# 10XGenomics/supernova

Measured on AMD Instinct MI355X. Metric: Gk-mers/s through count+graph at k=48, 1.2B×150bp; bit-exact counts, higher is better.
Workload: dtype u64

## Files before the change

### supernova_amd/csrc/snk_local.hip

```cpp
#include <string.h>
#include <cstring>
#include <rocprim/rocprim.hpp>

#include <type_traits>

#include "snk_ctx.h"
#include "snk_common.h"
#include "snk_kernels.h"
#include "snk_graph.h"
#include "snk_stages.h"

namespace {

constexpr uint32_t NONE = 0xFFFFFFFFu;
constexpr unsigned long long NONE64 = ~0ull;
constexpr uint16_t NONE16 = 0xFFFFu;
constexpr int TB = 256;

struct chunk_src {
    const uint32_t* chunk_n;
    const uint32_t* chunk_base;
    const uint4* extra;
    const unsigned long long* region_off;
    uint32_t NB, n_extra, n_regions;
    const uint8_t* span;
};
struct chunk_t {
    uint32_t bucket, n, lg, id;
    uint32_t span;
    uint64_t base;
};
struct bl_regions {
    const snk_u128* keys_r;
    const uint64_t* vals_r;
    const uint64_t* desc_src;
    snk_u128* keys_dense;
};
struct bl_shard {
    uint32_t bucket_base, NBl, me;
    uint32_t G;
    uint8_t* premote;
};
__global__ void __launch_bounds__(256) bl_chunk_merge_kernel(const uint32_t* __restrict__ chunk_n, const uint32_t* __restrict__ chunk_base, uint32_t NB, uint32_t G,
                                                             uint32_t cap, uint8_t* __restrict__ span, uint32_t* __restrict__ merged) {
    const uint32_t r = blockIdx.x * 256 + threadIdx.x;
    if (r >= G) return;
    uint32_t head = NONE, total = 0, m = 0, expect = 0;
    for (uint32_t b = r; b < NB; b += G) {
        const uint32_t n = chunk_n[b];
        span[b] = 1;
        merged[b] = n;
        if (n == 0) { head = NONE; continue; }
        const uint32_t base = chunk_base[b];
        if (head != NONE && base == expect && total + n <= cap && m < 255u) {
            total += n; ++m;
            merged[head] = total; merged[b] = 0; span[head] = (uint8_t)m;
        } else { head = b; total = n; m = 1; }
        expect = base + n;
    }
}
__global__ void __launch_bounds__(256) bl_chunk_desc_kernel(chunk_src cs, uint32_t nchunks, uint4* __restrict__ desc, uint64_t region_cap, uint64_t* __restrict__ desc_src) {
    const uint32_t c = blockIdx.x * 256 + threadIdx.x;
    if (c >= nchunks) return;
    uint32_t bucket, n, off = 0, meta = 0, region;
    if (c < cs.NB) {
        bucket = c; n = cs.chunk_n[c];
        if (n) off = cs.chunk_base[c];
        region = bucket % cs.n_regions;
        if (cs.span && n && cs.span[c] > 1) meta = 0x80000000u | cs.span[c];
    } else {
        const uint4 e = cs.extra[c - cs.NB];
        bucket = e.x; off = e.y; n = e.z & 0xFFFu; region = e.z >> 12; meta = e.w;
    }
    const uint64_t base = cs.region_off[region] + off;
    desc[c] = make_uint4((uint32_t)base, n, bucket, meta);
    if (desc_src) desc_src[c] = (uint64_t)region * region_cap + off;
}
__device__ __forceinline__ chunk_t chunk_get(const uint4* __restrict__ desc, uint32_t c) {
    const uint4 d = desc[c];
    chunk_t k;
    k.base = d.x; k.n = d.y; k.bucket = d.z; k.lg = d.w >> 24; k.id = d.w & 0xFFFFFFu; k.span = 1;
    if (d.w >> 31) { k.lg = 0; k.id = 0; k.span = d.w & 0xFFFFu; }
    return k;
}

__device__ __forceinline__ snk_kmer load_key(const snk_u128* keys, uint64_t i) {
    const uint64_t* p = reinterpret_cast<const uint64_t*>(keys + i);
    snk_kmer k;
    k.lo = p[0];
    k.hi = p[1];
    return k;
}
__device__ __forceinline__ uint32_t lhash(uint64_t hi, uint64_t lo) {
    uint32_t x = (uint32_t)(hi >> 32) * 0x9E3779B1u ^ (uint32_t)hi * 0x85EBCA77u ^ (uint32_t)(lo >> 32) * 0xC2B2AE3Du ^
                 (uint32_t)lo * 0x27D4EB2Fu;
    return snk_mix32(x);
}
template <int K>
__device__ __forceinline__ uint32_t oriented_base(snk_kmer k, bool rc, int idx) {
    return rc ? (snk_kmer_base<K>(k, K - 1 - idx) ^ 3u) : snk_kmer_base<K>(k, idx);
}

constexpr int BL_SPEC_LDS = 128;
constexpr int BL_SPEC_REPL = 64;
constexpr uint32_t BL_SPEC_BINS = 65536u;
constexpr uint32_t BL_SPEC_OVER = BL_SPEC_BINS + BL_SPEC_REPL * BL_SPEC_LDS / 2;
constexpr uint32_t BL_SPEC_WORDS = BL_SPEC_OVER + 16;
__global__ void __launch_bounds__(BL_SPEC_LDS) bl_spec_fold_kernel(unsigned long long* __restrict__ spec) {
    const uint32_t* rep = reinterpret_cast<const uint32_t*>(spec + BL_SPEC_BINS);
    unsigned long long s = 0;
    for (int r = 0; r < BL_SPEC_REPL; ++r) s += rep[r * BL_SPEC_LDS + threadIdx.x];
    spec[threadIdx.x] += s;
}
template <int K, int CAP, int T, bool BIG, bool GR, int MM>
__device__ __forceinline__ void bl_prune_chunk(const uint32_t c, const uint4* __restrict__ desc, uint32_t NB, bl_shard sh, const bl_regions& rg,
                                                     const snk_u128* __restrict__ keys, const uint64_t* __restrict__ vals,
                                                     uint32_t do_prune, uint8_t* __restrict__ ctx_out,
                                                     uint32_t* __restrict__ count_out, uint8_t* __restrict__ pend_out,
                                                     uint32_t* __restrict__ nbr_out, uint32_t* __restrict__ nbnd,
                                                     uint32_t* __restrict__ biglist, uint32_t* __restrict__ nbig,
                                                     unsigned long long* __restrict__ gindex, uint64_t gmask,
                                                     unsigned long long* __restrict__ spec, uint32_t* __restrict__ shist) {
    constexpr int HT = CAP <= 256 ? 512 : 4096;
    typedef typename std::conditional<(K <= 48 && !GR), uint32_t, uint64_t>::type klo_w;
    constexpr int KLS = (K <= 48 && !GR) ? 32 : 0;
    __shared__ uint64_t khi[CAP];
    __shared__ klo_w klo[CAP];
    __shared__ uint32_t ht[HT];
    __shared__ uint32_t bcnt;
    const int tid = threadIdx.x;
    const chunk_t ch = chunk_get(desc, c);
    if (ch.n == 0) return;
    if (!BIG && ch.n > (uint32_t)CAP) {
        if (tid == 0) biglist[atomicAdd(nbig, 1u)] = c;
        return;
    }
    const uint32_t n = ch.n;
    uint64_t src = ch.base;
    if (rg.keys_r) { src = rg.desc_src[c]; keys = rg.keys_r; vals = rg.vals_r; }
    __syncthreads();
    for (int s = tid; s < HT; s += T) ht[s] = 0;
    if (tid == 0) bcnt = 0;
    constexpr int NPT = (CAP + T - 1) / T;
    uint64_t myv[NPT];
    snk_kmer kq[NPT];
#pragma unroll
    for (int q = 0; q < NPT; ++q) {
        const uint32_t i = tid + q * T;
        myv[q] = 0;
        if (i < n) {
            kq[q] = load_key(keys, src + i);
            myv[q] = vals[src + i];
        }
    }
#pragma unroll
    for (int q = 0; q < NPT; ++q) {
        const uint32_t i = tid + q * T;
        if (i < n) {
            khi[i] = kq[q].hi;
            klo[i] = (klo_w)(kq[q].lo >> KLS);
            if (rg.keys_r) { uint64_t* d = reinterpret_cast<uint64_t*>(rg.keys_dense + ch.base + i); d[0] = kq[q].lo; d[1] = kq[q].hi; }
        }
    }
    __syncthreads();
    for (uint32_t i = tid; i < n; i += T) {
        uint32_t slot = lhash(khi[i], (uint64_t)klo[i] << KLS) & (HT - 1);
        for (;;) {
            const uint32_t old = atomicCAS(&ht[slot], 0u, i + 1u);
            if (old == 0u) break;
            slot = (slot + 1) & (HT - 1);
        }
    }
    __syncthreads();
    const uint32_t split_mask = (1u << ch.lg) - 1u;
    uint32_t mybnd = 0;
    __shared__ uint16_t mlist[8 * T];
    __shared__ uint32_t resL[T];
    __shared__ uint32_t mcnt;
#pragma unroll
    for (int q = 0; q < NPT; ++q) {
        const uint32_t i0 = q * T;
        if (i0 >= n) break;
        const uint32_t i = i0 + tid;
        const bool act = i < n;
        snk_kmer k;
        k.hi = act ? khi[i] : 0ull;
        k.lo = act ? ((uint64_t)klo[i] << KLS) : 0ull;
        uint64_t tag = 0;
        if (GR) { tag = k.lo & 0xFFFFFFFFull; k.lo &= ~0xFFFFFFFFull; }
        const uint64_t v = myv[q];
        const uint32_t c0 = (uint32_t)(v & 0xFFu);
        uint32_t keep = 0, miss = 0, nb0 = NONE, nb1 = NONE;
        const snk_kmer kr = snk_kmer_rc<K>(k);
        for (uint32_t rem = c0; rem; rem &= rem - 1) {
            const uint32_t bit = __ffs(rem) - 1;
            const snk_kmer y = bit < 4 ? snk_kmer_succ<K>(k, bit) : snk_kmer_pred<K>(k, bit - 4);
            const snk_kmer r = bit < 4 ? snk_kmer_pred<K>(kr, 3u - bit) : snk_kmer_succ<K>(kr, 7u - bit);
            const bool rev = snk_kmer_lt(r, y);
            snk_kmer cy = rev ? r : y;
            if (GR) cy.lo |= tag;
            int32_t j = -1;
            uint32_t slot = lhash(cy.hi, cy.lo) & (HT - 1);
            for (;;) {
                const uint32_t e = ht[slot];
                if (e == 0u) break;
                if (khi[e - 1] == cy.hi && ((uint64_t)klo[e - 1] << KLS) == cy.lo) { j = (int32_t)(e - 1); break; }
                slot = (slot + 1) & (HT - 1);
            }
            if (j >= 0) {
                keep |= 1u << bit;
                if (bit < 4) nb0 = ((uint32_t)j << 1) | (rev ? 1u : 0u); else nb1 = ((uint32_t)j << 1) | (rev ? 1u : 0u);
            } else miss |= 1u << bit;
        }
        if (tid == 0) mcnt = 0;
        resL[tid] = 0;
        __syncthreads();
        uint32_t pos = snk_wave_alloc(&mcnt, (uint32_t)__popc(miss));
        if (miss) {
            for (uint32_t bit = 0; bit < 8; ++bit)
                if (miss & (1u << bit)) mlist[pos++] = (uint16_t)((tid << 3) | bit);
        }
        __syncthreads();
        const uint32_t nm = mcnt;
        constexpr int SH = K - MM;
        constexpr int PER = (SH + 3) / 4;
        for (uint32_t it0 = 0; it0 < nm; it0 += T / 4) {
            const uint32_t item = it0 + (tid >> 2), sub = tid & 3u;
            const bool on = item < nm;
            const uint32_t ent = on ? mlist[item] : 0u;
            const uint32_t th = ent >> 3, bit = ent & 7u;
            const uint32_t ni = i0 + th;
            snk_kmer kk;
            kk.hi = on ? khi[ni] : 0ull;
            kk.lo = on ? ((uint64_t)klo[ni] << KLS) : 0ull;
            uint64_t ktag = 0;
            if (GR) { ktag = kk.lo & 0xFFFFFFFFull; kk.lo &= ~0xFFFFFFFFull; }
            const int first = bit < 4 ? 1 : 0;
            uint32_t mk = 0xFFFFFFFFu;
            for (int t = 0; t < PER; ++t) {
                const int sp = (int)sub * PER + t;
                if (sp < SH) {
                    const int pp = first + sp;
                    uint64_t w;
                    if (pp == 0) w = kk.hi;
                    else if (pp < 32) w = (kk.hi << (2 * pp)) | (kk.lo >> (64 - 2 * pp));
                    else if (pp == 32) w = kk.lo;
                    else w = kk.lo << (2 * pp - 64);
                    const uint32_t key = snk_mmer_key_top<MM>(w);
                    mk = key < mk ? key : mk;
                }
            }
            { const uint32_t o = __shfl_xor(mk, 1); mk = o < mk ? o : mk; }
            { const uint32_t o = __shfl_xor(mk, 2); mk = o < mk ? o : mk; }
            if (on && sub == 0) {
                const snk_kmer y = bit < 4 ? snk_kmer_succ<K>(kk, bit) : snk_kmer_pred<K>(kk, bit - 4);
                uint64_t wn;
                if (bit < 4) {
                    constexpr int pl = K - MM;
                    wn = pl < 32 ? ((y.hi << (2 * pl)) | (y.lo >> (64 - 2 * pl))) : (pl == 32 ? y.lo : (y.lo << (2 * pl - 64)));
                } else wn = y.hi;
                const uint32_t nkey = snk_mmer_key_top<MM>(wn);
                if (nkey < mk) mk = nkey;
                const uint32_t gb = snk_bucket_of_key(mk ^ (GR ? snk_group_mix((uint32_t)ktag) : 0u), NB);
                const uint32_t db = gb - (sh.bucket_base + ch.bucket);
                bool here = ch.span == 1 ? db == 0u : (gb >= sh.bucket_base + ch.bucket && db % sh.G == 0u && db / sh.G < ch.span);
                const bool remote = sh.NBl && gb / sh.NBl != sh.me;
                if (here && ch.lg) {
                    const snk_kmer r = snk_kmer_rc<K>(y);
                    snk_kmer cn = snk_kmer_lt(r, y) ? r : y;
                    if (GR) cn.lo |= ktag;
                    uint32_t h1, h2;
                    snk_kmer_hash_count<(K > 48) || GR>(cn, &h1, &h2);
                    here = (h2 & split_mask) == ch.id;
                }
                if (here && !(do_prune & 2u)) { if (!(do_prune & 1u)) atomicOr(&resL[th], 1u << bit); }
                else atomicOr(&resL[th], (1u << bit) | (0x100u << bit) | (remote ? (0x10000u << bit) : 0u));
            }
        }
        __syncthreads();
        const uint32_t res = resL[tid];
        keep |= res & 0xFFu;
        const uint32_t pm = (res >> 8) & 0xFFu;
        __syncthreads();
        if (!act) continue;
        const uint64_t gi = ch.base + i;
        ctx_out[gi] = (uint8_t)keep;
        pend_out[gi] = (uint8_t)pm;
        if (sh.premote) sh.premote[gi] = (uint8_t)(res >> 16);
        const uint32_t cnt = (uint32_t)(v >> 8);
        count_out[gi] = cnt;
        if (spec) {
            const uint32_t sc = cnt > 0xFFFFFFu ? 0xFFFFFFu : cnt;
            if (sc < (uint32_t)BL_SPEC_LDS) atomicAdd(&shist[sc], 1u);
            else if (sc < BL_SPEC_BINS) atomicAdd(&spec[sc], 1ull);
            else spec[BL_SPEC_OVER] = 1ull;
        }
        nbr_out[gi] = (nb0 == NONE ? 0x0FFFu : nb0) | (snk_kmer_eq(k, kr) ? 0x8000u : 0u) | ((nb1 == NONE ? 0x0FFFu : nb1) << 16);
        if (pm) {
            ++mybnd;
            if (gindex) {
                snk_kmer kk;
                kk.hi = khi[i];
                kk.lo = (uint64_t)klo[i] << KLS;
                uint32_t h1, h2;
                snk_kmer_hash2(kk, &h1, &h2);
                uint64_t slot = (((uint64_t)h1 << 32) | h2) & gmask;
                const unsigned long long ent = ((unsigned long long)h1 << 32) | (unsigned long long)(gi + 1);
                if (gindex[gmask + 1] == 0ull) {
                    bool placed = false;
                    for (uint32_t tries = 0; tries < 64; ++tries) {
                        const unsigned long long old = atomicCAS(&gindex[slot], 0ull, ent);
                        if (old == 0ull) { placed = true; break; }
                        slot = (slot + 1) & gmask;
                    }
                    if (!placed) gindex[gmask + 1] = 1ull;
                }
            }
        }
    }
    snk_wave_add(&bcnt, mybnd);
    __syncthreads();
    if (tid == 0) nbnd[c] = bcnt;
}
template <int K, int CAP, int T, bool BIG, bool GR, int MM>
__global__ void __launch_bounds__(T) bl_prune_kernel(const uint4* __restrict__ desc, uint32_t NB, bl_shard sh, bl_regions rg, const uint32_t* __restrict__ biglist_in,
                                                     uint32_t nchunks, uint32_t cpw,
                                                     const snk_u128* __restrict__ keys, const uint64_t* __restrict__ vals,
                                                     uint32_t do_prune, uint8_t* __restrict__ ctx_out,
                                                     uint32_t* __restrict__ count_out, uint8_t* __restrict__ pend_out,
                                                     uint32_t* __restrict__ nbr_out, uint32_t* __restrict__ nbnd,
                                                     uint32_t* __restrict__ biglist, uint32_t* __restrict__ nbig, const uint32_t* __restrict__ n_dev,
                                                     unsigned long long* __restrict__ gindex, uint64_t gmask, unsigned long long* __restrict__ spec) {
    __shared__ uint32_t shist[BL_SPEC_LDS];
    if (spec) {
        for (int j = threadIdx.x; j < BL_SPEC_LDS; j += T) shist[j] = 0;
        __syncthreads();
    }
    if (BIG && n_dev) {
        const uint32_t nb = *n_dev;
        for (uint32_t w = blockIdx.x; w < nb; w += gridDim.x)
            bl_prune_chunk<K, CAP, T, BIG, GR, MM>(biglist_in[w], desc, NB, sh, rg, keys, vals, do_prune, ctx_out, count_out, pend_out, nbr_out, nbnd, biglist, nbig, gindex, gmask,
                                                   spec, shist);
    } else {
        for (uint32_t r = 0; r < cpw; ++r) {
            const uint32_t w = blockIdx.x * cpw + r;
            if (w >= nchunks) break;
            bl_prune_chunk<K, CAP, T, BIG, GR, MM>(BIG ? biglist_in[w] : w, desc, NB, sh, rg, keys, vals, do_prune, ctx_out, count_out, pend_out, nbr_out,
                                           nbnd, biglist, nbig, gindex, gmask, spec, shist);
        }
    }
    if (spec) {
        __syncthreads();
        uint32_t* rep = reinterpret_cast<uint32_t*>(spec + BL_SPEC_BINS) + (blockIdx.x % BL_SPEC_REPL) * BL_SPEC_LDS;
        for (int j = threadIdx.x; j < BL_SPEC_LDS; j += T)
            if (shist[j]) atomicAdd(&rep[j], shist[j]);
    }
}

__global__ void __launch_bounds__(TB) bl_index_build_kernel(const snk_u128* __restrict__ keys, const uint8_t* __restrict__ pend,
                                                            uint64_t n, unsigned long long* __restrict__ tab, uint64_t mask) {
    const uint64_t i = (uint64_t)blockIdx.x * TB + threadIdx.x;
    if (i >= n || !pend[i]) return;
    const snk_kmer k = load_key(keys, i);
    uint32_t h1, h2;
    snk_kmer_hash2(k, &h1, &h2);
    uint64_t slot = (((uint64_t)h1 << 32) | h2) & mask;
    const unsigned long long ent = ((unsigned long long)h1 << 32) | (unsigned long long)(i + 1);
    for (;;) {
        const unsigned long long old = atomicCAS(&tab[slot], 0ull, ent);
        if (old == 0ull) break;
        slot = (slot + 1) & mask;
    }
}
template <int K, bool GR>
__global__ void __launch_bounds__(TB) bl_resolve_kernel(const snk_u128* __restrict__ keys, const uint8_t* __restrict__ pend,
                                                        uint64_t n, const unsigned long long* __restrict__ tab, uint64_t mask,
                                                        uint32_t do_prune, uint8_t* __restrict__ ctx, uint32_t* __restrict__ rq,
                                                        const uint8_t* __restrict__ premote) {
    constexpr int SPAN = 8 * TB;
    __shared__ uint16_t list[SPAN];
    __shared__ uint32_t cnt;
    const uint64_t base = (uint64_t)blockIdx.x * SPAN;
    if (threadIdx.x == 0) cnt = 0;
    __syncthreads();
    {
        const uint64_t i8 = base + 8ull * threadIdx.x;
        unsigned long long w = 0;
        if (i8 + 8 <= n) w = *reinterpret_cast<const unsigned long long*>(pend + i8);
        else for (uint64_t q = i8; q < n; ++q) w |= (unsigned long long)pend[q] << (8 * (q - i8));
        if (w) {
            uint32_t m = 0;
            for (int q = 0; q < 8; ++q) if ((w >> (8 * q)) & 0xFFull) ++m;
            uint32_t pos = atomicAdd(&cnt, m);
            for (int q = 0; q < 8; ++q) if ((w >> (8 * q)) & 0xFFull) list[pos++] = (uint16_t)(8 * threadIdx.x + q);
        }
    }
    __syncthreads();
    const uint32_t m = cnt;
    for (uint32_t it = threadIdx.x; it < m; it += TB) {
        const uint64_t i = base + list[it];
        const uint32_t pm = pend[i] & (premote ? ~(uint32_t)premote[i] : 0xFFu);
        snk_kmer k = load_key(keys, i);
        uint64_t tag = 0;
        if (GR) { tag = k.lo & 0xFFFFFFFFull; k.lo &= ~0xFFFFFFFFull; }
        uint32_t c = ctx[i];
        const snk_kmer kr = snk_kmer_rc<K>(k);
        for (uint32_t rem = pm; rem; rem &= rem - 1) {
            const uint32_t bit = __ffs(rem) - 1;
            const snk_kmer y = bit < 4 ? snk_kmer_succ<K>(k, bit) : snk_kmer_pred<K>(k, bit - 4);
            const snk_kmer r = bit < 4 ? snk_kmer_pred<K>(kr, 3u - bit) : snk_kmer_succ<K>(kr, 7u - bit);
            const bool rev = snk_kmer_lt(r, y);
            snk_kmer cy = rev ? r : y;
            if (GR) cy.lo |= tag;
            uint32_t h1, h2;
            snk_kmer_hash2(cy, &h1, &h2);
            uint64_t slot = (((uint64_t)h1 << 32) | h2) & mask;
            int64_t j = -1;
            for (;;) {
                const unsigned long long e = tab[slot];
                if (e == 0ull) break;
                if ((uint32_t)(e >> 32) == h1) {
                    const uint64_t idx = (uint32_t)e - 1u;
                    if (snk_kmer_eq(load_key(keys, idx), cy)) { j = (int64_t)idx; break; }
                }
                slot = (slot + 1) & mask;
            }
            if (j >= 0) rq[2 * i + (bit >> 2)] = ((uint32_t)j << 1) | (rev ? 1u : 0u);
            else if (do_prune) c &= ~(1u << bit);
            else rq[2 * i + (bit >> 2)] = NONE;
        }
        ctx[i] = (uint8_t)c;
    }
}

struct bl_extra_pool {
    unsigned long long* cur;
    uint64_t f0, b0;
    uint64_t fcap, bcap;
};
struct bl_dist_args {
    const uint8_t* premote;
    const uint32_t* rq_idx;
    const uint16_t* rq_meta;
    const unsigned long long* node_off;
    unsigned long long my_node_off;
};
template <int K, int CAP, int T, bool BIG, bool EMIT, bool DIST, bool GR>
__global__ void __launch_bounds__(T) bl_frag_kernel(const uint4* __restrict__ desc, const uint32_t* __restrict__ biglist_in,
                                                    const snk_u128* __restrict__ keys, const uint8_t* __restrict__ ctx,
                                                    const uint8_t* __restrict__ pend, const uint32_t* __restrict__ nbr,
                                                    const uint32_t* __restrict__ rq, bl_dist_args da, uint32_t* __restrict__ nfrag,
                                                    const uint32_t* __restrict__ foff, const uint64_t* __restrict__ boff,
                                                    uint32_t* __restrict__ nk, unsigned long long* __restrict__ hl_self,
                                                    unsigned long long* __restrict__ hl_nb, uint64_t* __restrict__ bstart,
                                                    uint8_t* __restrict__ fbases, uint32_t* __restrict__ fgroup, uint32_t* __restrict__ sfrag, bl_extra_pool xp) {
    constexpr int SPT = (2 * CAP + T - 1) / T;
    constexpr int NPT = (CAP + T - 1) / T;
    constexpr bool ONEW = T == 64;
    typedef typename std::conditional<(K <= 48 && !GR), uint32_t, uint64_t>::type klo_w;
    constexpr int KLS = (K <= 48 && !GR) ? 32 : 0;
    __shared__ uint64_t khi[ONEW ? 1 : CAP];
    __shared__ klo_w klo[ONEW ? 1 : CAP];
    __shared__ uint16_t nbL[2 * CAP];
    typedef typename std::conditional<(CAP <= 256), uint32_t, uint64_t>::type wrec_t;
    constexpr int FB = CAP <= 256 ? 10 : 16;
    constexpr uint32_t FM = (1u << FB) - 1u;
    __shared__ uint16_t lnk[2 * CAP];
    __shared__ wrec_t wr[2 * CAP];
    constexpr bool WIDE = (uint32_t)CAP * (uint32_t)K > 65535u;
    uint16_t* foffL = nbL;
    __shared__ uint32_t frel[WIDE ? CAP : 1];
    __shared__ uint16_t hnode[CAP];
    __shared__ uint8_t ctxL[CAP], pendL[CAP];
    __shared__ uint32_t fcnt, bcnt, changed;
    const int tid = threadIdx.x;
    const uint32_t c = BIG ? biglist_in[blockIdx.x] : blockIdx.x;
    const chunk_t ch = chunk_get(desc, c);
    if (ch.n == 0) return;
    if (!BIG && ch.n > (uint32_t)CAP) return;
    const uint32_t n = ch.n;
    const uint32_t c_foff = EMIT ? foff[c] : 0u;
    const uint64_t c_boff = EMIT ? boff[c] : 0ull;
    if constexpr (!ONEW) {
        if (tid == 0) { fcnt = 0; bcnt = 0; changed = 0; }
    }
    uint32_t w_frags = 0, w_bases = 0;
    snk_kmer kq[NPT] = {};
    {
        uint32_t cq[NPT], pq[NPT];
        uint32_t nq[NPT];
#pragma unroll
        for (int q = 0; q < NPT; ++q) {
            const uint32_t i = tid + q * T;
            if (i < n) {
                const uint64_t gi = ch.base + i;
                if (EMIT) kq[q] = load_key(keys, gi);
                cq[q] = ctx[gi];
                pq[q] = pend[gi];
                nq[q] = nbr[gi];
            }
        }
#pragma unroll
        for (int q = 0; q < NPT; ++q) {
            const uint32_t i = tid + q * T;
            if (i < n) {
                if constexpr (EMIT && !ONEW) {
                    const snk_kmer k = kq[q];
                    khi[i] = k.hi;
                    klo[i] = (klo_w)(k.lo >> KLS);
                }
                ctxL[i] = (uint8_t)cq[q];
                pendL[i] = (uint8_t)pq[q];
                nbL[2 * i] = (uint16_t)(nq[q] & 0x8FFFu);
                nbL[2 * i + 1] = (uint16_t)((nq[q] >> 16) & 0x0FFFu);
            }
        }
    }
    __syncthreads();
    auto is_pal = [&](uint32_t i) -> bool { return (nbL[2 * i] >> 15) != 0; };
    auto key_of = [&](uint32_t i) -> snk_kmer {
        snk_kmer k;
        if constexpr (ONEW) {
            k = load_key(keys, ch.base + i);
            k.lo = (k.lo >> KLS) << KLS;
        } else {
            k.hi = khi[i];
            k.lo = (uint64_t)klo[i] << KLS;
        }
        return k;
    };
    auto own_key = [&](int q, uint32_t i) -> snk_kmer {
        if constexpr (ONEW) return kq[q];
        else return key_of(i);
    };
    uint32_t myterm = 0;
    for (uint32_t s = tid; s < 2 * n; s += T) {
        const uint32_t i = s >> 1, side = s & 1u;
        const uint32_t cc = ctxL[i];
        const uint32_t bits = side ? (cc >> 4) : (cc & 15u);
        uint16_t out = NONE16;
        if (__popc(bits) == 1) {
            const uint32_t b = __ffs(bits) - 1;
            if (!((pendL[i] >> (4 * side + b)) & 1u)) {
                const uint32_t nb = nbL[s] & 0x0FFFu;
                if (nb != 0x0FFFu) {
                    const uint32_t j = nb >> 1, rev = nb & 1u;
                    const uint32_t fs = side ^ 1u ^ rev;
                    const uint32_t cj = ctxL[j];
                    const uint32_t deg = fs ? __popc(cj & 0xF0u) : __popc(cj & 0x0Fu);
                    if (deg == 1 && !is_pal(i) && !is_pal(j)) out = (uint16_t)((j << 1) | fs);
                }
            }
        }
        lnk[s] = out;
        if (!EMIT) { if (out == NONE16) ++myterm; }
        else if (out == NONE16) wr[s] = (wrec_t)FM | ((wrec_t)s << (2 * FB));
        else wr[s] = (wrec_t)(out ^ 1u) | ((wrec_t)1 << FB) | ((wrec_t)(out ^ 1u) << (2 * FB));
    }
    if (!EMIT) {
        if constexpr (ONEW) {
            const uint32_t total = (uint32_t)__builtin_amdgcn_readlane((int)snk_wave_scan_incl(myterm), 63);
            if (tid == 0) nfrag[c] = total >> 1;
        } else {
            snk_wave_add(&fcnt, myterm);
            __syncthreads();
            if (tid == 0) nfrag[c] = fcnt >> 1;
        }
        return;
    }
    __syncthreads();
    int max_rounds = 2;
    while ((1u << (max_rounds - 1)) < 2 * n) ++max_rounds;
    for (int round = 0; round < max_rounds; ++round) {
        wrec_t rr[SPT];
        bool any = false;
#pragma unroll
        for (int q = 0; q < SPT; ++q) {
            if ((uint32_t)(q * T) >= 2 * n) break;
            const uint32_t s = tid + q * T;
            if (s < 2 * n) {
                const wrec_t a0 = wr[s];
                const uint32_t n1 = (uint32_t)a0 & FM;
                rr[q] = a0;
                if (n1 != FM) {
                    const wrec_t a1 = wr[n1];
                    const uint32_t d = (((uint32_t)(a0 >> FB) & FM) + ((uint32_t)(a1 >> FB) & FM)) & FM;
                    rr[q] = (a1 & (wrec_t)FM) | ((wrec_t)d << FB) | (a1 & ((wrec_t)FM << (2 * FB)));
                    any = true;
                }
            }
        }
        if constexpr (ONEW) {
            if (!__any(any)) break;
        }
        __syncthreads();
#pragma unroll
        for (int q = 0; q < SPT; ++q) {
            if ((uint32_t)(q * T) >= 2 * n) break;
            const uint32_t s = tid + q * T;
            if (s < 2 * n) wr[s] = rr[q];
        }
        if constexpr (ONEW) {
            __syncthreads();
        } else {
            if (any) changed = 1;
            __syncthreads();
            const bool go = changed != 0;
            __syncthreads();
            if (tid == 0) changed = 0;
            if (!go) break;
        }
    }
    __syncthreads();
    auto w_next = [&](uint32_t st) -> uint32_t { return (uint32_t)wr[st] & FM; };
    auto w_dist = [&](uint32_t st) -> uint32_t { return (uint32_t)(wr[st] >> FB) & FM; };
    auto w_tail = [&](uint32_t st) -> uint32_t { return (uint32_t)(wr[st] >> (2 * FB)) & FM; };

    auto half_link = [&](uint32_t s) -> unsigned long long {
        const uint32_t i = s >> 1, side = s & 1u;
        const uint32_t cc = ctxL[i];
        const uint32_t bits = side ? (cc >> 4) : (cc & 15u);
        if (__popc(bits) != 1 || is_pal(i)) return NONE64;
        const uint32_t b = __ffs(bits) - 1;
        if (!((pendL[i] >> (4 * side + b)) & 1u)) return NONE64;
        snk_kmer k = key_of(i);
        if (GR) k.lo &= ~0xFFFFFFFFull;
        const snk_kmer y = side ? snk_kmer_pred<K>(k, b) : snk_kmer_succ<K>(k, b);
        if (snk_kmer_eq(y, snk_kmer_rc<K>(y))) return NONE64;
// ... 627 lines not shown
```

Baseline: 101.2.

## Shrink prune kernel LDS and registers for single-wave blocks to raise occupancy

For non-BIG 64-thread blocks, the local hash table now stores 16-bit indices (half the LDS), and the miss list is capped at 128 entries and processed in batches. Wave-level scans replace shared-memory atomic counters. Values are now streamed one iteration ahead instead of held in a per-thread array, and a waves_per_eu attribute asks the compiler to keep register use low enough for higher occupancy. The costs are a read-then-CAS loop on packed 16-bit slots, extra batch loops when misses exceed the list cap, and possible register spills from the occupancy constraint.

Result: faster. 102.5 (median of 6 runs) (+1.3%).

```diff
diff --git a/supernova_amd/csrc/snk_local.hip b/supernova_amd/csrc/snk_local.hip
--- a/supernova_amd/csrc/snk_local.hip
+++ b/supernova_amd/csrc/snk_local.hip
@@ -124,9 +124,11 @@
     constexpr int HT = CAP <= 256 ? 512 : 4096;
     typedef typename std::conditional<(K <= 48 && !GR), uint32_t, uint64_t>::type klo_w;
     constexpr int KLS = (K <= 48 && !GR) ? 32 : 0;
+    constexpr bool ONE = !BIG && T == 64;
+    constexpr int ML = ONE ? 128 : 8 * T;
     __shared__ uint64_t khi[CAP];
     __shared__ klo_w klo[CAP];
-    __shared__ uint32_t ht[HT];
+    __shared__ uint32_t ht[ONE ? HT / 2 : HT];
     __shared__ uint32_t bcnt;
     const int tid = threadIdx.x;
     const chunk_t ch = chunk_get(desc, c);
@@ -139,48 +141,54 @@
     uint64_t src = ch.base;
     if (rg.keys_r) { src = rg.desc_src[c]; keys = rg.keys_r; vals = rg.vals_r; }
     __syncthreads();
-    for (int s = tid; s < HT; s += T) ht[s] = 0;
-    if (tid == 0) bcnt = 0;
+    for (int s = tid; s < (ONE ? HT / 2 : HT); s += T) ht[s] = 0;
+    if constexpr (!ONE) { if (tid == 0) bcnt = 0; }
     constexpr int NPT = (CAP + T - 1) / T;
-    uint64_t myv[NPT];
-    snk_kmer kq[NPT];
+    {
+        snk_kmer kq[NPT];
 #pragma unroll
-    for (int q = 0; q < NPT; ++q) {
-        const uint32_t i = tid + q * T;
-        myv[q] = 0;
-        if (i < n) {
-            kq[q] = load_key(keys, src + i);
-            myv[q] = vals[src + i];
-        }
-    }
+        for (int q = 0; q < NPT; ++q) {
+            const uint32_t i = tid + q * T;
+            if (i < n) kq[q] = load_key(keys, src + i);
+        }
 #pragma unroll
-    for (int q = 0; q < NPT; ++q) {
-        const uint32_t i = tid + q * T;
-        if (i < n) {
-            khi[i] = kq[q].hi;
-            klo[i] = (klo_w)(kq[q].lo >> KLS);
-            if (rg.keys_r) { uint64_t* d = reinterpret_cast<uint64_t*>(rg.keys_dense + ch.base + i); d[0] = kq[q].lo; d[1] = kq[q].hi; }
-        }
-    }
+        for (int q = 0; q < NPT; ++q) {
+            const uint32_t i = tid + q * T;
+            if (i < n) {
+                khi[i] = kq[q].hi;
+                klo[i] = (klo_w)(kq[q].lo >> KLS);
+                if (rg.keys_r) { uint64_t* d = reinterpret_cast<uint64_t*>(rg.keys_dense + ch.base + i); d[0] = kq[q].lo; d[1] = kq[q].hi; }
+            }
+        }
+    }
+    uint64_t vnext = (uint32_t)tid < n ? vals[src + tid] : 0ull;
     __syncthreads();
     for (uint32_t i = tid; i < n; i += T) {
         uint32_t slot = lhash(khi[i], (uint64_t)klo[i] << KLS) & (HT - 1);
-        for (;;) {
-            const uint32_t old = atomicCAS(&ht[slot], 0u, i + 1u);
-            if (old == 0u) break;
-            slot = (slot + 1) & (HT - 1);
+        if constexpr (ONE) {
+            for (;;) {
+                uint32_t* const w = &ht[slot >> 1];
+                const uint32_t s16 = (slot & 1u) << 4;
+                const uint32_t cur = *reinterpret_cast<volatile uint32_t*>(w);
+                if ((cur >> s16) & 0xFFFFu) { slot = (slot + 1) & (HT - 1); continue; }
+                if (atomicCAS(w, cur, cur | ((i + 1u) << s16)) == cur) break;
+            }
+        } else {
+            for (;;) {
+                const uint32_t old = atomicCAS(&ht[slot], 0u, i + 1u);
+                if (old == 0u) break;
+                slot = (slot + 1) & (HT - 1);
+            }
         }
     }
     __syncthreads();
     const uint32_t split_mask = (1u << ch.lg) - 1u;
     uint32_t mybnd = 0;
-    __shared__ uint16_t mlist[8 * T];
+    __shared__ uint16_t mlist[ML];
     __shared__ uint32_t resL[T];
     __shared__ uint32_t mcnt;
-#pragma unroll
-    for (int q = 0; q < NPT; ++q) {
-        const uint32_t i0 = q * T;
-        if (i0 >= n) break;
+    const uint16_t* const ht16 = reinterpret_cast<const uint16_t*>(ht);
+    for (uint32_t i0 = 0; i0 < n; i0 += T) {
         const uint32_t i = i0 + tid;
         const bool act = i < n;
         snk_kmer k;
@@ -188,7 +196,8 @@
         k.lo = act ? ((uint64_t)klo[i] << KLS) : 0ull;
         uint64_t tag = 0;
         if (GR) { tag = k.lo & 0xFFFFFFFFull; k.lo &= ~0xFFFFFFFFull; }
-        const uint64_t v = myv[q];
+        const uint64_t v = vnext;
+        vnext = i + T < n ? vals[src + i + T] : 0ull;
         const uint32_t c0 = (uint32_t)(v & 0xFFu);
         uint32_t keep = 0, miss = 0, nb0 = NONE, nb1 = NONE;
         const snk_kmer kr = snk_kmer_rc<K>(k);
@@ -202,7 +211,7 @@
             int32_t j = -1;
             uint32_t slot = lhash(cy.hi, cy.lo) & (HT - 1);
             for (;;) {
-                const uint32_t e = ht[slot];
+                const uint32_t e = ONE ? (uint32_t)ht16[slot] : ht[slot];
                 if (e == 0u) break;
                 if (khi[e - 1] == cy.hi && ((uint64_t)klo[e - 1] << KLS) == cy.lo) { j = (int32_t)(e - 1); break; }
                 slot = (slot + 1) & (HT - 1);
@@ -212,70 +221,82 @@
                 if (bit < 4) nb0 = ((uint32_t)j << 1) | (rev ? 1u : 0u); else nb1 = ((uint32_t)j << 1) | (rev ? 1u : 0u);
             } else miss |= 1u << bit;
         }
-        if (tid == 0) mcnt = 0;
+        if constexpr (!ONE) { if (tid == 0) mcnt = 0; }
         resL[tid] = 0;
         __syncthreads();
-        uint32_t pos = snk_wave_alloc(&mcnt, (uint32_t)__popc(miss));
-        if (miss) {
-            for (uint32_t bit = 0; bit < 8; ++bit)
-                if (miss & (1u << bit)) mlist[pos++] = (uint16_t)((tid << 3) | bit);
-        }
-        __syncthreads();
-        const uint32_t nm = mcnt;
+        const uint32_t nmiss = (uint32_t)__popc(miss);
+        uint32_t pos, total = 0;
+        if constexpr (ONE) {
+            const uint32_t incl = snk_wave_scan_incl(nmiss);
+            total = (uint32_t)__builtin_amdgcn_readlane((int)incl, 63);
+            pos = incl - nmiss;
+        } else pos = snk_wave_alloc(&mcnt, nmiss);
         constexpr int SH = K - MM;
         constexpr int PER = (SH + 3) / 4;
-        for (uint32_t it0 = 0; it0 < nm; it0 += T / 4) {
-            const uint32_t item = it0 + (tid >> 2), sub = tid & 3u;
-            const bool on = item < nm;
-            const uint32_t ent = on ? mlist[item] : 0u;
-            const uint32_t th = ent >> 3, bit = ent & 7u;
-            const uint32_t ni = i0 + th;
-            snk_kmer kk;
-            kk.hi = on ? khi[ni] : 0ull;
-            kk.lo = on ? ((uint64_t)klo[ni] << KLS) : 0ull;
-            uint64_t ktag = 0;
-            if (GR) { ktag = kk.lo & 0xFFFFFFFFull; kk.lo &= ~0xFFFFFFFFull; }
-            const int first = bit < 4 ? 1 : 0;
-            uint32_t mk = 0xFFFFFFFFu;
-            for (int t = 0; t < PER; ++t) {
-                const int sp = (int)sub * PER + t;
-                if (sp < SH) {
-                    const int pp = first + sp;
-                    uint64_t w;
-                    if (pp == 0) w = kk.hi;
-                    else if (pp < 32) w = (kk.hi << (2 * pp)) | (kk.lo >> (64 - 2 * pp));
-                    else if (pp == 32) w = kk.lo;
-                    else w = kk.lo << (2 * pp - 64);
-                    const uint32_t key = snk_mmer_key_top<MM>(w);
-                    mk = key < mk ? key : mk;
+        for (uint32_t base = 0;; base += ML) {
+            {
+                uint32_t e = pos - base;
+                for (uint32_t rem = miss; rem; rem &= rem - 1, ++e)
+                    if (e < (uint32_t)ML) mlist[e] = (uint16_t)((tid << 3) | (__ffs(rem) - 1));
+            }
+            __syncthreads();
+            if constexpr (!ONE) total = mcnt;
+            const uint32_t nm = total - base < (uint32_t)ML ? total - base : (uint32_t)ML;
+            for (uint32_t it0 = 0; it0 < nm; it0 += T / 4) {
+                const uint32_t item = it0 + (tid >> 2), sub = tid & 3u;
+                const bool on = item < nm;
+                const uint32_t ent = on ? mlist[item] : 0u;
+                const uint32_t th = ent >> 3, bit = ent & 7u;
+                const uint32_t ni = i0 + th;
+                snk_kmer kk;
+                kk.hi = on ? khi[ni] : 0ull;
+                kk.lo = on ? ((uint64_t)klo[ni] << KLS) : 0ull;
+                uint64_t ktag = 0;
+                if (GR) { ktag = kk.lo & 0xFFFFFFFFull; kk.lo &= ~0xFFFFFFFFull; }
+                const int first = bit < 4 ? 1 : 0;
+                uint32_t mk = 0xFFFFFFFFu;
+                for (int t = 0; t < PER; ++t) {
+                    const int sp = (int)sub * PER + t;
+                    if (sp < SH) {
+                        const int pp = first + sp;
+                        uint64_t w;
+                        if (pp == 0) w = kk.hi;
+                        else if (pp < 32) w = (kk.hi << (2 * pp)) | (kk.lo >> (64 - 2 * pp));
+                        else if (pp == 32) w = kk.lo;
+                        else w = kk.lo << (2 * pp - 64);
+                        const uint32_t key = snk_mmer_key_top<MM>(w);
+                        mk = key < mk ? key : mk;
+                    }
                 }
-            }
-            { const uint32_t o = __shfl_xor(mk, 1); mk = o < mk ? o : mk; }
-            { const uint32_t o = __shfl_xor(mk, 2); mk = o < mk ? o : mk; }
-            if (on && sub == 0) {
-                const snk_kmer y = bit < 4 ? snk_kmer_succ<K>(kk, bit) : snk_kmer_pred<K>(kk, bit - 4);
-                uint64_t wn;
-                if (bit < 4) {
-                    constexpr int pl = K - MM;
-                    wn = pl < 32 ? ((y.hi << (2 * pl)) | (y.lo >> (64 - 2 * pl))) : (pl == 32 ? y.lo : (y.lo << (2 * pl - 64)));
-                } else wn = y.hi;
-                const uint32_t nkey = snk_mmer_key_top<MM>(wn);
-                if (nkey < mk) mk = nkey;
-                const uint32_t gb = snk_bucket_of_key(mk ^ (GR ? snk_group_mix((uint32_t)ktag) : 0u), NB);
-                const uint32_t db = gb - (sh.bucket_base + ch.bucket);
-                bool here = ch.span == 1 ? db == 0u : (gb >= sh.bucket_base + ch.bucket && db % sh.G == 0u && db / sh.G < ch.span);
-                const bool remote = sh.NBl && gb / sh.NBl != sh.me;
-                if (here && ch.lg) {
-                    const snk_kmer r = snk_kmer_rc<K>(y);
-                    snk_kmer cn = snk_kmer_lt(r, y) ? r : y;
-                    if (GR) cn.lo |= ktag;
-                    uint32_t h1, h2;
-                    snk_kmer_hash_count<(K > 48) || GR>(cn, &h1, &h2);
-                    here = (h2 & split_mask) == ch.id;
+                { const uint32_t o = __shfl_xor(mk, 1); mk = o < mk ? o : mk; }
+                { const uint32_t o = __shfl_xor(mk, 2); mk = o < mk ? o : mk; }
+                if (on && sub == 0) {
+                    const snk_kmer y = bit < 4 ? snk_kmer_succ<K>(kk, bit) : snk_kmer_pred<K>(kk, bit - 4);
+                    uint64_t wn;
+                    if (bit < 4) {
+                        constexpr int pl = K - MM;
+                        wn = pl < 32 ? ((y.hi << (2 * pl)) | (y.lo >> (64 - 2 * pl))) : (pl == 32 ? y.lo : (y.lo << (2 * pl - 64)));
+                    } else wn = y.hi;
+                    const uint32_t nkey = snk_mmer_key_top<MM>(wn);
+                    if (nkey < mk) mk = nkey;
+                    const uint32_t gb = snk_bucket_of_key(mk ^ (GR ? snk_group_mix((uint32_t)ktag) : 0u), NB);
+                    const uint32_t db = gb - (sh.bucket_base + ch.bucket);
+                    bool here = ch.span == 1 ? db == 0u : (gb >= sh.bucket_base + ch.bucket && db % sh.G == 0u && db / sh.G < ch.span);
+                    const bool remote = sh.NBl && gb / sh.NBl != sh.me;
+                    if (here && ch.lg) {
+                        const snk_kmer r = snk_kmer_rc<K>(y);
+                        snk_kmer cn = snk_kmer_lt(r, y) ? r : y;
+                        if (GR) cn.lo |= ktag;
+                        uint32_t h1, h2;
+                        snk_kmer_hash_count<(K > 48) || GR>(cn, &h1, &h2);
+                        here = (h2 & split_mask) == ch.id;
+                    }
+                    if (here && !(do_prune & 2u)) { if (!(do_prune & 1u)) atomicOr(&resL[th], 1u << bit); }
+                    else atomicOr(&resL[th], (1u << bit) | (0x100u << bit) | (remote ? (0x10000u << bit) : 0u));
                 }
-                if (here && !(do_prune & 2u)) { if (!(do_prune & 1u)) atomicOr(&resL[th], 1u << bit); }
-                else atomicOr(&resL[th], (1u << bit) | (0x100u << bit) | (remote ? (0x10000u << bit) : 0u));
-            }
+            }
+            if (base + ML >= total) break;
+            __syncthreads();
         }
         __syncthreads();
         const uint32_t res = resL[tid];
@@ -318,12 +339,19 @@
             }
         }
     }
-    snk_wave_add(&bcnt, mybnd);
-    __syncthreads();
-    if (tid == 0) nbnd[c] = bcnt;
-}
+    if constexpr (ONE) {
+        const uint32_t b = (uint32_t)__builtin_amdgcn_readlane((int)snk_wave_scan_incl(mybnd), 63);
+        if (tid == 0) nbnd[c] = b;
+    } else {
+        snk_wave_add(&bcnt, mybnd);
+        __syncthreads();
+        if (tid == 0) nbnd[c] = bcnt;
+    }
+}
+template <int K, bool BIG, bool GR, int MM>
+constexpr int bl_prune_waves = BIG ? 1 : (K <= 48 && !GR) ? (MM <= 16 ? 8 : 7) : 6;
 template <int K, int CAP, int T, bool BIG, bool GR, int MM>
-__global__ void __launch_bounds__(T) bl_prune_kernel(const uint4* __restrict__ desc, uint32_t NB, bl_shard sh, bl_regions rg, const uint32_t* __restrict__ biglist_in,
+__global__ void __launch_bounds__(T) __attribute__((amdgpu_waves_per_eu(bl_prune_waves<K, BIG, GR, MM>, 8))) bl_prune_kernel(const uint4* __restrict__ desc, uint32_t NB, bl_shard sh, bl_regions rg, const uint32_t* __restrict__ biglist_in,
                                                      uint32_t nchunks, uint32_t cpw,
                                                      const snk_u128* __restrict__ keys, const uint64_t* __restrict__ vals,
                                                      uint32_t do_prune, uint8_t* __restrict__ ctx_out,
```
